# skywaLKer518/A-Recsys

Measured on AMD Instinct MI355X. Metric: training interactions/sec + sampled-negatives/sec, dim-128, 1/2/4/8 MI355X, higher is better.
Workload: dtype f32; 1 GPU; C3 (BASELINE configs[2]): id feature + multi-hot category attribute, HET layout (two tables, ~20 tokens/item over 100 k rows); synthetic 1000000-item/1000000-user HMF, dim 128, WMRB 'mw' loss, 1024 shared negatives/step (pool redrawn on device every 50 step...; batch=16384, n_sampled=1024, dim=128, n_items=1000000, hipgraph=True, ids_fed_from=HBM (device-resident ring of batches)

## Files before the change

### a-recsys_amd/csrc/scorer.hip

```cpp
#include "common.h"
#include "posmask.h"

namespace arx {

namespace {

typedef __bf16 bf16x8 __attribute__((ext_vector_type(8)));
typedef float f32x16 __attribute__((ext_vector_type(16)));

#ifndef SC_TRACE_CHUNKS
#define SC_TRACE_CHUNKS 0
#endif
#ifdef SC_TRACE
__device__ unsigned long long g_sc_trace[4096];
#define SC_T(ev_)                                                                                        \
  if (blockIdx.x == (gridDim.x > 5 ? 5 : 0) && threadIdx.x == 0 && tcount < 4096)                        \
    g_sc_trace[tcount++] = ((unsigned long long)(ev_) << 56) | (__builtin_readcyclecounter() & 0xFFFFFFFFFFFFFFull);
#define SC_TDECL int tcount = 0;
#define SC_TREAL(ev_)                  \
  if (blockIdx.x == (gridDim.x > 5 ? 5 : 0) && threadIdx.x == 0 && tcount < 4096)                        \
    g_sc_trace[tcount++] = ((unsigned long long)(ev_) << 56) | (__builtin_amdgcn_s_memrealtime() & 0xFFFFFFFFFFFFFFull);
#else
#define SC_TREAL(ev_)
#define SC_T(ev_)
#define SC_TDECL
#endif
constexpr int kScHits = 8;
constexpr int kScSlots = 4;
constexpr int kScAhead = 3;
constexpr int kScStageBytes = 3 * 32 * 256;

typedef __bf16 sc_bf2 __attribute__((ext_vector_type(2)));
typedef float sc_f2 __attribute__((ext_vector_type(2)));
__device__ __forceinline__ void split3x2(float x, float y, uint32_t& p1, uint32_t& p2, uint32_t& p3) {
  p1 = __builtin_bit_cast(uint32_t, __builtin_convertvector((sc_f2){x, y}, sc_bf2));
  const float rx = x - __uint_as_float(p1 << 16), ry = y - __uint_as_float(p1 & 0xFFFF0000u);
  p2 = __builtin_bit_cast(uint32_t, __builtin_convertvector((sc_f2){rx, ry}, sc_bf2));
  const float sx = rx - __uint_as_float(p2 << 16), sy = ry - __uint_as_float(p2 & 0xFFFF0000u);
  p3 = __builtin_bit_cast(uint32_t, __builtin_convertvector((sc_f2){sx, sy}, sc_bf2));
}

#ifdef SC_ABL_NOBAR
// ... 91 lines not shown
}

__device__ __forceinline__ float sc_wsum(float v) {
#pragma unroll
  for (int o = 32; o > 0; o >>= 1) v += __shfl_xor(v, o, 64);
  return v;
}

struct ScTScore {
  const float* U; int64_t ldu;
  const float* T; int64_t ldt;
  const float* tb; int64_t tb_stride;
  float* tscore; float* tscore2;
};

template <bool MASKS>
__global__ __launch_bounds__(256) void k_sc_prep(const float* __restrict__ P, int64_t ldp, int64_t S, int d,
                                                 const float* __restrict__ pbias, uint16_t* __restrict__ Pp,
                                                 uint16_t* __restrict__ PT, int64_t ldpt, float* __restrict__ pool_bad,
                                                 PosMask pm,
                                                 int64_t mask_rows, int64_t B, int32_t* __restrict__ hits,
                                                 int32_t* __restrict__ nhit, const float* __restrict__ seq_w,
                                                 int64_t seq_rows, float* __restrict__ row_w_out, ScTScore ts,
                                                 uint32_t* __restrict__ maskR, int64_t ldr) {
  __shared__ float tile[32 * 129];
  __shared__ float sbad[4];
  const int tid = threadIdx.x;
  const int64_t pblocks = S / 32;
  const int64_t hblocks = (B + 7) / 8;
  if ((int64_t)blockIdx.x >= pblocks + hblocks) {
    float* part = tile;
    const int cx = tid & 31, ty = tid >> 5;
    const int64_t b = ((int64_t)blockIdx.x - pblocks - hblocks) * 32 + cx;
    const int64_t L = B / seq_rows;
    float sum = 0.f;
    if (b < seq_rows)
      for (int64_t t = ty; t < L; t += 8) sum += seq_w[t * seq_rows + b];
// ... 28 lines not shown
    __syncthreads();
    if (tid == 0) pool_bad[blockIdx.x] = (sbad[0] + sbad[1]) + (sbad[2] + sbad[3]);
    sc_emit_planes_t(tile, ld, 32, d, PT, (int64_t)d * ldpt, ldpt, r0, tid, 256);
    return;
  }
  const int lane = tid & 63, hl = lane & 31;
  const int64_t r = (((int64_t)blockIdx.x - pblocks) * 256 + tid) >> 5;
  const bool valid = r < B;
  float4 u4 = make_float4(0.f, 0.f, 0.f, 0.f), t4 = u4;
  if (valid && 4 * hl < d) {
    u4 = *reinterpret_cast<const float4*>(ts.U + r * ts.ldu + 4 * hl);
    t4 = *reinterpret_cast<const float4*>(ts.T + r * ts.ldt + 4 * hl);
  }
  const float tbv = (valid && ts.tb) ? ts.tb[r * ts.tb_stride] : 0.f;
  const bool walker = valid && r < mask_rows;
  const int64_t reps = walker ? (B - r + mask_rows - 1) / mask_rows : 0;
  const int usr = walker ? pm.user_ids[r % mask_rows] : 0;
  const int beg = walker ? pm.pos_ptr[usr] : 0, end = walker ? pm.pos_ptr[usr + 1] : 0;
  int n = 0;
  uint32_t mw0 = 0u, mw1 = 0u;
  for (int p0 = beg;; p0 += 32) {
    const bool active = p0 < end && (MASKS || n >= 0);
    if (!__any(active)) break;
    const int p = p0 + hl;
    int j = -1;
    if (active && p < end) {
      j = pos_slot(pm, pm.pos_items[p]);
      if (j < 0 || j >= S) j = -1;
    }
    const unsigned long long hm64 = __ballot(j >= 0);
    uint32_t hm = (lane >> 5) ? (uint32_t)(hm64 >> 32) : (uint32_t)hm64;
    if (MASKS) {
      while (__any(hm != 0u)) {
        const bool some = hm != 0u;
        const int srcl = some ? __builtin_ctz(hm) : 0;
        hm &= hm - 1u;
        const int jj = __shfl(j, (lane & 32) + srcl, 64);
        if (some && hl == ((jj >> 5) & 31)) {
          if (jj < 1024) mw0 |= 1u << (jj & 31);
          else mw1 |= 1u << (jj & 31);
        }
      }
    } else {
      const int k = __popc(hm);
      if (active && n >= 0) {
        if (n + k > kScHits) n = -1;
        else {
          if (j >= 0) {
            const int at = n + __popc(hm & ((1u << hl) - 1u));
            for (int64_t t = 0; t < reps; ++t) hits[(r + t * mask_rows) * kScHits + at] = j;
          }
          n += k;
        }
      }
    }
  }
  if (MASKS && walker) {
    const int nwords = (int)(S >> 5);
    if (hl < nwords) maskR[(int64_t)hl * ldr + r] = mw0;
    if (hl + 32 < nwords) maskR[(int64_t)(hl + 32) * ldr + r] = mw1;
  }
  float dot = u4.x * t4.x + u4.y * t4.y + u4.z * t4.z + u4.w * t4.w;
#pragma unroll
  for (int o = 16; o > 0; o >>= 1) dot += __shfl_xor(dot, o, 64);
  if (!MASKS && hl == 0)
    for (int64_t t = 0; t < reps; ++t) nhit[r + t * mask_rows] = n;
  if (hl == 0 && valid) {
    const float t = dot + tbv;
    ts.tscore[r] = t;
    if (ts.tscore2) ts.tscore2[r] = t;
  }
}

template <int KD>
__global__ __launch_bounds__(512) void k_sc_hinge(int64_t B, int64_t S, int CW, const float* __restrict__ U, int64_t ldu,
                                                  const float* __restrict__ tscore,
                                                  const uint16_t* __restrict__ Pp, const float* __restrict__ bias,
                                                  uint32_t* __restrict__ bits, int64_t ldbits, float* __restrict__ rs_part,
                                                  float* __restrict__ cnt_part) {
  constexpr int NCH = KD / 16;
  constexpr int ROWB = KD * 2;
  constexpr int TPS = 256 / ROWB;
  constexpr int TILEB = 3 * 32 * ROWB;
  extern __shared__ __attribute__((aligned(1024))) char lds[];
  float* sbias = reinterpret_cast<float*>(lds + kScSlots * kScStageBytes);
  uint32_t* swords = reinterpret_cast<uint32_t*>(sbias + CW);
  const int tid = threadIdx.x;
  const int lane = tid & 63;
  const int wv = tid >> 6;
  const int nsplit = (int)(S / CW);
  int64_t rb;
  int ch;
// ... 18 lines not shown
    sc_loader_loop<ROWB>(ld, lds, nstage);
    return;
  }

  const int lr = lane & 31, kg = lane >> 5;
  const int64_t row = rb * 128 + wv * 32 + lr;
  const bool ok = row < B;
  SC_TDECL
  SC_TREAL(120)
  SC_T(99)
  bf16x8 a1[NCH], a2[NCH], a3[NCH];
  float4 ru[NCH][2];
  float tm1;
  {
    float bv[2];
#pragma unroll
    for (int k = 0; k < 2; ++k) bv[k] = (bias && tid + 256 * k < CW) ? bias[col0 + tid + 256 * k] : 0.f;
    tm1 = (ok ? tscore[row] : 0.f) - 1.f;
    const float* up = U + (ok ? row : 0) * ldu + 8 * kg;
#pragma unroll
    for (int c = 0; c < NCH; ++c) {
      ru[c][0] = *reinterpret_cast<const float4*>(up + 16 * c);
      ru[c][1] = *reinterpret_cast<const float4*>(up + 16 * c + 4);
      if (c & 1) __builtin_amdgcn_sched_barrier(0);
    }
#pragma unroll
    for (int k = 0; k < 2; ++k)
      if (tid + 256 * k < CW) sbias[tid + 256 * k] = bv[k];
  }
#define SC_SPLIT(c_)                                                                                     \
  {                                                                                                      \
    uint32_t p1[4], p2[4], p3[4];                                                                        \
    split3x2(ru[c_][0].x, ru[c_][0].y, p1[0], p2[0], p3[0]);                                             \
    split3x2(ru[c_][0].z, ru[c_][0].w, p1[1], p2[1], p3[1]);                                             \
    split3x2(ru[c_][1].x, ru[c_][1].y, p1[2], p2[2], p3[2]);                                             \
    split3x2(ru[c_][1].z, ru[c_][1].w, p1[3], p2[3], p3[3]);                                             \
    a1[c_] = __builtin_bit_cast(bf16x8, make_uint4(p1[0], p1[1], p1[2], p1[3]));                         \
    a2[c_] = __builtin_bit_cast(bf16x8, make_uint4(p2[0], p2[1], p2[2], p2[3]));                         \
    a3[c_] = __builtin_bit_cast(bf16x8, make_uint4(p3[0], p3[1], p3[2], p3[3]));                         \
  }
  SC_SPLIT(0)
  float rs = 0.f;
  int cnt = 0;
  constexpr bool FA1 = ROWB == 256;
  uint32_t fa[FA1 ? 1 : NCH];
#pragma unroll
  for (int c = 0; c < (FA1 ? 1 : NCH); ++c) fa[c] = (uint32_t)(lr * ROWB + 16 * ((2 * c + kg) ^ sc_swz<ROWB>(lr)));
#define SC_FA(c_) (FA1 ? (fa[0] ^ (uint32_t)((c_) << 5)) : fa[FA1 ? 0 : (c_)])

  f32x16 hiA, loA, hiB, loB;
  constexpr int VPC = 16 / NCH;
  constexpr int VPM = KD == 128 ? 2 : 4;
  uint32_t* wptr = swords + wv * 32 + lr;
  uint4 fr[4][3];
  float4 bvn[4];
  uint32_t h = 0u;
  float zero_v;
  asm volatile("v_mov_b32 %0, 0" : "=v"(zero_v));
#ifndef SC_PF
#define SC_PF 1
#endif
  static_assert(SC_PF == 1 || !FA1, "the single address register steps to the next image one chunk ahead");
#define SC_LD3(set_, c_)                                                                                 \
  {                                                                                                      \
    const uint32_t fa_ = SC_FA(c_);                                                                      \
    fr[set_][0] = *reinterpret_cast<const uint4*>(lds + fa_);                                            \
    fr[set_][1] = *reinterpret_cast<const uint4*>(lds + fa_ + 32 * ROWB);                                \
    fr[set_][2] = *reinterpret_cast<const uint4*>(lds + fa_ + 64 * ROWB);                                \
  }
#define SC_MFMA6(hi_, lo_, c_)                                                                           \
  lo_ = SC_MFMA(b3, a1[c_], lo_);                                                                        \
  hi_ = SC_MFMA(b1, a1[c_], hi_);                                                                        \
  lo_ = SC_MFMA(b1, a3[c_], lo_);                                                                        \
  lo_ = SC_MFMA(b2, a2[c_], lo_);                                                                        \
  lo_ = SC_MFMA(b2, a1[c_], lo_);                                                                        \
  lo_ = SC_MFMA(b1, a2[c_], lo_);
#define SC_WORD(hw_, j_)                                                                                 \
  {                                                                                                      \
    const uint32_t hh = (hw_) & 0xFFFFu;                                                                 \
    cnt += __popc(hh);                                                                                   \
    const uint32_t w = ((hh & 0xFu) | ((hh & 0xF0u) << 4) | ((hh & 0xF00u) << 8) | ((hh & 0xF000u) << 12)) << (4 * kg); \
    const auto sw = __builtin_amdgcn_permlane32_swap(w, w, false, false);                                \
    wptr[(j_) * 128] = sw[0] | sw[1];                                                                    \
  }
#ifdef SC_ABL_NOEPI
#define SC_EPI_ON(x_) false
#else
#define SC_EPI_ON(x_) (x_)
#endif
#ifndef SC_EPI_C0
#define SC_EPI_C0 0
#endif
#ifndef SC_EPI_V
#define SC_EPI_V VPC
#endif
#ifdef SC_ABL_EPI_NOREAD
#define SC_EPI_READ(x_) (bvn[i >> 2].x + tm1)
#else
// ... 16 lines not shown
    __builtin_amdgcn_sched_group_barrier(0x008, 2, 0);                                                   \
  }
#else
#define SC_CHUNK_SCHED(c_)                                                                               \
  _Pragma("unroll") for (int m = 0; m < 6; ++m) {                                                        \
    __builtin_amdgcn_sched_group_barrier(0x008, 1, 0);                                                   \
    if ((c_) == 0) __builtin_amdgcn_sched_group_barrier(0x002, VPM + 3, 0);                              \
    else __builtin_amdgcn_sched_group_barrier(0x002, VPM, 0);                                            \
  }
#endif
#define SC_CHUNK_SCHED_PRO                                                                               \
  _Pragma("unroll") for (int m = 0; m < 6; ++m) {                                                        \
    __builtin_amdgcn_sched_group_barrier(0x008, 1, 0);                                                   \
    __builtin_amdgcn_sched_group_barrier(0x002, 8, 0);                                                   \
  }
#define SC_TILE(hi_, lo_, hy_, ly_, EPI_, PRO_, jw_, jb0_, jb_, dl_, BAR_)                               \
  {                                                                                                      \
    const uint32_t dl = (uint32_t)(dl_);                                                                 \
    _Pragma("unroll") for (int c = 0; c < NCH; ++c) {                                                    \
      if ((BAR_) && c == NCH / 2) sc_barrier();                                                          \
      const bf16x8 b1 = __builtin_bit_cast(bf16x8, fr[c % 4][0]), b2 = __builtin_bit_cast(bf16x8, fr[c % 4][1]), \
                   b3 = __builtin_bit_cast(bf16x8, fr[c % 4][2]);                                        \
      if (FA1 && c == NCH - 1) fa[0] += dl;         \
      SC_LD3((c + SC_PF) % 4, (c + SC_PF) % NCH)    \
       \
       \
                         \
      _Pragma("unroll") for (int g = 0; g < 4; ++g) {                                                    \
        const int lastc = SC_EPI_C0 + (15 - 4 * g) / SC_EPI_V;           \
        if (lastc + 1 < NCH ? c == lastc + 1 : c == 0)                                                   \
          bvn[g] = *reinterpret_cast<const float4*>(sbias + (lastc + 1 < NCH ? (jb_) : (jb0_)) * 32 + 4 * kg + 8 * g); \
      }                                                                                                  \
      __builtin_amdgcn_sched_barrier(0);                                                                 \
      SC_MFMA6(hi_, lo_, c)                                                                              \
      if (!FA1) fa[FA1 ? 0 : c] += dl;                                                                   \
      if (c == 0 && (jw_) >= 0) {                                                                        \
        const uint32_t hw = h;                                                                           \
        SC_WORD(hw, jw_)                                                                                 \
      }                                                                                                  \
      if (SC_EPI_ON(EPI_) && c >= SC_EPI_C0 && c < SC_EPI_C0 + 16 / SC_EPI_V) {                          \
        _Pragma("unroll") for (int q = 0; q < SC_EPI_V; ++q) {                                           \
          const int i = 15 - ((c - SC_EPI_C0) * SC_EPI_V + q);                                           \
          const float nv = SC_EPI_READ(-hy_[i] - ly_[i]);                                                \
          h = __builtin_amdgcn_alignbit(h, __float_as_uint(nv), 31);                                     \
          rs += fmaxf(-nv, 0.f);                                                                         \
          const float4 bq = bvn[i >> 2];                                                                 \
          SC_EPI_WRITE(hy_[i] = ((i & 3) == 0 ? bq.x : (i & 3) == 1 ? bq.y : (i & 3) == 2 ? bq.z : bq.w) - tm1;) \
          SC_EPI_WRITE({ float z_; asm volatile("v_mov_b32 %0, 0" : "=v"(z_)); ly_[i] = z_; })          \
        }                                                                                                \
      }                                                                                                  \
      if ((PRO_) && c + 1 < NCH) { SC_SPLIT(c + 1) }                                                     \
      if (PRO_) { SC_CHUNK_SCHED_PRO } else { SC_CHUNK_SCHED(c) }                                        \
      __builtin_amdgcn_sched_barrier(0);                                                                 \
      if (SC_TRACE_CHUNKS || c == NCH - 1) { SC_T(1 + c) }                                               \
    }                                                                                                    \
  }
#define SC_INIT(hi_, lo_, j_)                                                                            \
  {                                                                                                      \
    const float* bt = sbias + (j_) * 32 + 4 * kg;                                                        \
    _Pragma("unroll") for (int g = 0; g < 4; ++g) {                                                      \
      const float4 bv = *reinterpret_cast<const float4*>(bt + 8 * g);                                    \
      hi_[4 * g] = bv.x - tm1; hi_[4 * g + 1] = bv.y - tm1; hi_[4 * g + 2] = bv.z - tm1; hi_[4 * g + 3] = bv.w - tm1; \
    }                                                                                                    \
    _Pragma("unroll") for (int e = 0; e < 16; ++e) lo_[e] = zero_v;                                      \
  }
  auto img = [&](int j) -> int { return ((j / TPS) % kScSlots) * kScStageBytes + (j % TPS) * TILEB; };
  auto step = [&](int j) -> int { return img(j + 1) - img(j); };
  SC_T(100)
  sc_barrier();
  SC_T(101)
  SC_INIT(hiA, loA, 0)
  SC_INIT(hiB, loB, 1)
#pragma unroll
  for (int c = 0; c < SC_PF; ++c) SC_LD3(c, c)
  auto tcl = [&](int j) -> int { return j < ntile ? j : ntile - 1; };
  SC_TILE(hiA, loA, hiB, loB, false, true, -1, tcl(1), tcl(2), step(0), TPS == 1)
  SC_TILE(hiB, loB, hiA, loA, true, false, -1, tcl(2), tcl(3), step(1), true)
  for (int j = 2; j + 1 < ntile; j += 2) {
    SC_TILE(hiA, loA, hiB, loB, true, false, j - 2, tcl(j + 1), tcl(j + 2), step(j), TPS == 1)
    SC_TILE(hiB, loB, hiA, loA, true, false, j - 1, tcl(j + 2), tcl(j + 3), step(j + 1), true)
  }
  SC_WORD(h, ntile - 2)
#pragma unroll
  for (int i = 15; i >= 0; --i) {
    const float nv = -hiB[i] - loB[i];
    h = __builtin_amdgcn_alignbit(h, __float_as_uint(nv), 31);
    rs += fmaxf(-nv, 0.f);
  }
  SC_WORD(h, ntile - 1)
  SC_T(110)
  asm volatile("s_waitcnt lgkmcnt(0)" ::: "memory");
  if (ok) {
    for (int j = kg; j < ntile; j += 2) bits[(col0 / 32 + j) * ldbits + row] = swords[j * 128 + wv * 32 + lr];
  }
  SC_T(111)
  SC_TREAL(121)
#undef SC_LD3
#undef SC_SPLIT
#undef SC_MFMA6
#undef SC_TILE
#undef SC_WORD
#undef SC_INIT
  rs += __shfl_xor(rs, 32, 64);
  cnt += __shfl_xor(cnt, 32, 64);
  if (kg == 0 && ok) {
    rs_part[(int64_t)ch * B + row] = rs;
    cnt_part[(int64_t)ch * B + row] = (float)cnt;
  }
}

struct ScRows {
  const float* rs_part;
  const float* cnt_part;
  int nsplit;
  uint32_t* bits;
  int64_t ldbits;
  uint32_t* bitsT; int64_t ldbt;
  const float* tscore;
  const float* U; int64_t ldu;
  const float* T; int64_t ldt;
  const float* P; int64_t ldp;
  const float* pb;
  int d;
  float gscale;
  const float* row_w;
  float* batch_loss;
  float* g_out;
  float* dtscore; int64_t dts_stride;
  float* dU; int64_t lddu;
  float* dT; int64_t lddt;
  uint16_t* UgT; int64_t ldug;
  float* dbp;
  const int32_t* hits;
  const int32_t* nhit;
  const float* pool_bad;
};

template <int LPR>
__global__ __launch_bounds__(512) void k_sc_rows_g(ScRows a, PosMask pm, int64_t mask_rows, int64_t B, int64_t S) {
  constexpr int G = 64 / LPR;
  constexpr int WPL = 64 / LPR;
  constexpr int ROUNDS = 4 / G;
  static_assert(G == 2 || G == 4, "d = 128 or d = 64");
  __shared__ float tile[32 * 129];
  __shared__ uint32_t sbits[32 * 64];
  __shared__ float sg[32];
  const int tid = threadIdx.x;
  const int lane = tid & 63;
  const int wv = tid >> 6;
  const int j = lane % LPR, grp = lane / LPR, gbase = grp * LPR;
  const int64_t r0 = (int64_t)blockIdx.x * 32;
  const int nwords = (int)(S >> 5);
  const int ld = a.d + 1;
  const float pbad = sc_wsum(lane < nwords ? a.pool_bad[lane] : 0.f);
  auto gsum = [](float v) {
#pragma unroll
    for (int o = LPR / 2; o > 0; o >>= 1) v += __shfl_xor(v, o, 64);
    return v;
  };
#pragma unroll
  for (int it = 0; it < ROUNDS; ++it) {
    const int rl = wv * 4 + it * G + grp;
    const int64_t r = r0 + rl;
    const bool live = r < B;
    float4 uq = make_float4(0.f, 0.f, 0.f, 0.f), tq = uq;
    float sq = 0.f, cq = 0.f, t = 0.f;
    int nh = 0;
    uint32_t w[WPL], w0[WPL];
#pragma unroll
    for (int k = 0; k < WPL; ++k) w[k] = 0u;
    if (live) {
      for (int p = 0; p < a.nsplit; ++p) {
        sq += a.rs_part[(int64_t)p * B + r];
        cq += a.cnt_part[(int64_t)p * B + r];
      }
      t = a.tscore[r];
      uq = *reinterpret_cast<const float4*>(a.U + r * a.ldu + j * 4);
      tq = *reinterpret_cast<const float4*>(a.T + r * a.ldt + j * 4);
      nh = a.nhit[r];
#pragma unroll
      for (int k = 0; k < WPL; ++k)
        if (k * LPR + j < nwords) w[k] = a.bits[(int64_t)(k * LPR + j) * a.ldbits + r];
    }
#pragma unroll
    for (int k = 0; k < WPL; ++k) w0[k] = w[k];
    if (__any(live && nh != 0)) {
      auto take_out = [&](int jj, bool act) {
        const int wi = jj >> 5, own = wi % LPR, slot = wi / LPR;
        uint32_t mine = w[0];
#pragma unroll
        for (int k = 1; k < WPL; ++k) mine = slot == k ? w[k] : mine;
        const uint32_t word = __shfl(mine, gbase + own, 64);
        const bool on = act && ((word >> (jj & 31)) & 1u);
        float4 pr = make_float4(0.f, 0.f, 0.f, 0.f);
        if (on) pr = *reinterpret_cast<const float4*>(a.P + (int64_t)jj * a.ldp + j * 4);
        const float x = gsum(uq.x * pr.x + uq.y * pr.y + uq.z * pr.z + uq.w * pr.w) + ((on && a.pb) ? a.pb[jj] : 0.f);
        const float v = x - t + 1.f;
        if (on) {
          sq -= v > 0.f ? v : 0.f;
          cq -= 1.f;
          if (j == own) {
#pragma unroll
            for (int k = 0; k < WPL; ++k)
              if (slot == k) w[k] &= ~(1u << (jj & 31));
          }
        }
      };
      const bool listed = live && nh > 0;
      const int myhit = (listed && j < nh) ? a.hits[r * kScHits + j] : 0;
      for (int k = 0; k < kScHits; ++k) {
        const bool act = listed && k < nh;
        if (!__any(act)) break;
        take_out(__shfl(myhit, gbase + k, 64), act);
      }
      const bool walk = live && nh < 0;
      if (__any(walk)) {
        const int usr = walk ? pm.user_ids[r % mask_rows] : 0;
        const int beg = walk ? pm.pos_ptr[usr] : 0, end = walk ? pm.pos_ptr[usr + 1] : 0;
        for (int p0 = beg;; p0 += LPR) {
          const bool more = walk && p0 < end;
          if (!__any(more)) break;
          const int p = p0 + j;
          int js = -1;
          if (more && p < end) {
            js = pos_slot(pm, pm.pos_items[p]);
            if (js < 0 || js >= S) js = -1;
          }
          const unsigned long long bal = __ballot(js >= 0);
          uint32_t hm = (uint32_t)((bal >> gbase) & ((LPR == 32) ? 0xffffffffull : 0xffffull));
          while (__any(hm != 0u)) {
            const bool act = hm != 0u;
            const int src = act ? __builtin_ctz(hm) : 0;
            hm &= hm - 1u;
            take_out(__shfl(js, gbase + src, 64), act);
          }
        }
      }
      if (live && nh != 0) {
#pragma unroll
        for (int k = 0; k < WPL; ++k)
          if (k * LPR + j < nwords && w[k] != w0[k]) a.bits[(int64_t)(k * LPR + j) * a.ldbits + r] = w[k];
      }
    }
    sq = fmaxf(sq, 0.f) + (pbad + gsum(((uq.x + uq.y) + (uq.z + uq.w) + (tq.x + tq.y) + (tq.z + tq.w)) * 0.f) + t * 0.f);
    const float g = live ? a.gscale * (a.row_w ? a.row_w[r] : 1.f) / (1.f + sq) : 0.f;
    const float dt = -g * cq;
    if (j == 0) {
      sg[rl] = g;
      if (live) {
        if (a.batch_loss) a.batch_loss[r] = logf(1.f + sq);
        if (a.dtscore) a.dtscore[r * a.dts_stride] = dt;
      }
      a.g_out[r] = g;
    }
#pragma unroll
    for (int k = 0; k < WPL; ++k)
      if (k * LPR + j < nwords) sbits[rl * 64 + k * LPR + j] = w[k];
// ... 690 lines not shown
    float* tp = tile + rl * (D + 1) + c4;
    const float cu = live ? coef : 0.f;
    tp[0] = cu * u.x; tp[1] = cu * u.y; tp[2] = cu * u.z; tp[3] = cu * u.w;
  }
  __syncthreads();
  sc_emit_planes_t(tile, D + 1, 32, D, a.UgT, (int64_t)D * a.ldug, a.ldug, r0, tid, 256);
}


}

struct ScLayout {
  int64_t Bp, ldbits, ldbt, nblk;
  int64_t ldpt, ldug;
  int nsplit, CW;
  size_t bits, bitsT, g, t, rs, cnt, hits, nhit, Pp, PT, UgT, dbp, pbad, total;
};

static bool sc_layout(int64_t B, int64_t S, int d, ScLayout* L) {
  if (!(d == 64 || d == 128) || S % 128 != 0 || S < 128 || S > 2048 || B < 1) return false;
  L->Bp = (B + 127) / 128 * 128;
  L->ldbits = (B + 255) / 256 * 256;
  L->ldbt = (S + 255) / 256 * 256;
  L->nblk = L->Bp / 32;
  L->ldpt = S + 128;
  L->ldug = L->Bp + 128;
  L->CW = S >= 1024 ? 512 : (S >= 256 ? (int)(S / 2) : (int)S);
  L->nsplit = (int)(S / L->CW);
  size_t o = 0;
  auto take = [&](size_t bytes) { const size_t at = o; o += al256(bytes); return at; };
  L->bits = take((size_t)(S / 32) * L->ldbits * 4);
  L->bitsT = take((size_t)L->nblk * L->ldbt * 4);
  L->g = take((size_t)L->Bp * 4);
  L->t = take((size_t)B * 4);
  L->rs = take((size_t)L->nsplit * B * 4);
  L->cnt = take((size_t)L->nsplit * B * 4);
  L->hits = take((size_t)B * kScHits * 4);
  L->nhit = take((size_t)B * 4);
  L->Pp = take((size_t)3 * S * d * 2);
  L->PT = take((size_t)3 * d * L->ldpt * 2);
  L->UgT = take((size_t)3 * d * L->ldug * 2);
  L->dbp = take((size_t)L->nblk * S * 4);
  L->pbad = take(64 * 4);
  L->total = o;
  return true;
}

static int sc_raise_lds() {
  const int cap = 160 * 1024;
  ARX_CHECK_HIP(hipFuncSetAttribute(reinterpret_cast<const void*>(k_sc_hinge<128>), hipFuncAttributeMaxDynamicSharedMemorySize, cap));
  ARX_CHECK_HIP(hipFuncSetAttribute(reinterpret_cast<const void*>(k_sc_hinge<64>), hipFuncAttributeMaxDynamicSharedMemorySize, cap));
  ARX_CHECK_HIP(hipFuncSetAttribute(reinterpret_cast<const void*>(k_sc_bits<false>), hipFuncAttributeMaxDynamicSharedMemorySize, cap));
  ARX_CHECK_HIP(hipFuncSetAttribute(reinterpret_cast<const void*>(k_sc_bits<true>), hipFuncAttributeMaxDynamicSharedMemorySize, cap));
  return ARX_OK;
}

}

// ... 47 lines not shown
  if (!ok) {
    set_error("arx_mw_scorer_fwd: shape not supported (d in {64, 128}, S %% 128 == 0, 128 <= S <= 2048, 16-byte rows)");
    return ARX_EUNSUPPORTED;
  }
  if (state_bytes < L.total) {
    set_error("arx_mw_scorer_fwd: state too small (%zu < %zu)", state_bytes, L.total);
    return ARX_EWORKSPACE;
  }
  if (int rc = sc_raise_lds()) return rc;
  hipStream_t s = as_stream(stream);
  char* st = reinterpret_cast<char*>(state);
  uint32_t* bits = reinterpret_cast<uint32_t*>(st + L.bits);
  float* t = reinterpret_cast<float*>(st + L.t);
  float* rs_part = reinterpret_cast<float*>(st + L.rs);
  float* cnt_part = reinterpret_cast<float*>(st + L.cnt);
  int32_t* hits = reinterpret_cast<int32_t*>(st + L.hits);
  int32_t* nhit = reinterpret_cast<int32_t*>(st + L.nhit);
  uint16_t* Pp = reinterpret_cast<uint16_t*>(st + L.Pp);
  uint16_t* PT = reinterpret_cast<uint16_t*>(st + L.PT);
  const PosMask pm = make_pos_mask(user_ids, pos_ptr, pos_items, item2slot);
  const int64_t mrows = mask_rows > 0 ? mask_rows : B;
  if (phases & 1) {
    const int64_t grid = S / 32 + ceil_div(B, 8) + (seq_w ? ceil_div(seq_rows, 32) : 0);
    const ScTScore ts{U, ldu, T, ldt, tbias, tb_stride > 0 ? tb_stride : 1, t, tscore_out};
    k_sc_prep<false><<<(int)grid, 256, 0, s>>>(P, ldp, S, d, pbias, Pp, PT, L.ldpt, reinterpret_cast<float*>(st + L.pbad),
                                               pm, mrows, B, hits, nhit, seq_w, seq_rows, row_w, ts, nullptr, 0);
    ARX_CHECK_LAUNCH();
  }
  if (phases & 2) {
    const int64_t grid = ceil_div(B, 128) * L.nsplit;
    const size_t lds = (size_t)kScSlots * kScStageBytes + (size_t)L.CW * 4 + (size_t)(L.CW / 32) * 128 * 4;
    if (d == 128)
      k_sc_hinge<128><<<(int)grid, 512, lds, s>>>(B, S, L.CW, U, ldu, t, Pp, pbias, bits, L.ldbits, rs_part, cnt_part);
    else
      k_sc_hinge<64><<<(int)grid, 512, lds, s>>>(B, S, L.CW, U, ldu, t, Pp, pbias, bits, L.ldbits, rs_part, cnt_part);
    ARX_CHECK_LAUNCH();
  }
  if (phases & 4) {
    ScRows a{rs_part, cnt_part, L.nsplit, bits, L.ldbits, reinterpret_cast<uint32_t*>(st + L.bitsT), L.ldbt, t, U, ldu, T, ldt,
             P, ldp, pbias, d, gscale, row_w, batch_loss, reinterpret_cast<float*>(st + L.g), dtscore,
             dtscore_stride > 0 ? dtscore_stride : 1, dU, lddu, dT, lddt, reinterpret_cast<uint16_t*>(st + L.UgT), L.ldug,
             reinterpret_cast<float*>(st + L.dbp), hits, nhit, reinterpret_cast<const float*>(st + L.pbad)};
    if (d == 64) k_sc_rows_g<16><<<(int)L.nblk, 512, 0, s>>>(a, pm, mrows, B, S);
    else k_sc_rows_g<32><<<(int)L.nblk, 512, 0, s>>>(a, pm, mrows, B, S);
    ARX_CHECK_LAUNCH();
  }
  return ARX_OK;
}

int arx_mw_scorer_bwd_du(int64_t B, int64_t S, int d, const void* state, float beta, float* dU, int64_t lddu,
                         void* stream) {
  ScLayout L;
  ARX_CHECK_ARG(state && dU && sc_layout(B, S, d, &L), "arx_mw_scorer_bwd_du: bad argument / shape");
  ARX_CHECK_ARG(lddu % 4 == 0 && lddu >= d && (reinterpret_cast<uintptr_t>(dU) & 15) == 0,
                "arx_mw_scorer_bwd_du: dU rows must be 16-byte aligned");
  if (int rc = sc_raise_lds()) return rc;
  const char* st = reinterpret_cast<const char*>(state);
  const int64_t grid = ceil_div(B, 256) * (d / 32);
  k_sc_bits<false><<<(int)grid, 512, (size_t)kScSlots * (kScStageBytes + 4096), as_stream(stream)>>>(
// ... 62 lines not shown
      part, (int)nsl, S, d, beta, dI, lddi, dbp, L.nblk, db, dbblocks, batch_loss, row_w, B, gscale, loss_out,
      stepblocks, bps, Lsteps, db_steps);
  ARX_CHECK_LAUNCH();
  return ARX_OK;
}

}

namespace arx {
namespace {

struct McLayout {
  int64_t Bp, ldpt, ldug, ldr;
  int nsplit;
  int64_t CW;
  size_t maskR, mask_bytes, t, tneg, coef, rs, O, hits, nhit, Pp, PT, Up, UgT, pbad, zeros, total;
};

bool mc_layout(int64_t B, int64_t S, int d, McLayout* L) {
  if (!(d == 64 || d == 128) || S % 128 != 0 || S < 128 || S > 2048 || B < 1) return false;
  L->Bp = (B + 127) / 128 * 128;
  L->ldpt = S + 128;
  L->ldug = L->Bp + 128;
  L->ldr = L->Bp;
  int ns = 1;
  while (ns < 4 && (L->Bp / 128) * ns < 3 * (int64_t)cu_count() && S / (2 * ns) >= 128 && (S / (2 * ns)) % 32 == 0) ns *= 2;
  L->nsplit = ns;
  L->CW = S / ns;
  size_t o = 0;
  auto take = [&](size_t bytes) { const size_t at = o; o += al256(bytes); return at; };
  L->maskR = take((size_t)(S / 32) * L->ldr * 4);
  L->mask_bytes = o;
  L->t = take((size_t)B * 4);
  L->tneg = take((size_t)L->Bp * 4);
  L->coef = take((size_t)L->Bp * 4);
  L->rs = take((size_t)ns * B * 4);
  L->O = take((size_t)ns * L->Bp * d * 4);
  L->hits = take((size_t)B * kScHits * 4);
  L->nhit = take((size_t)B * 4);
  L->Pp = take((size_t)3 * S * d * 2);
  L->PT = take((size_t)3 * d * L->ldpt * 2);
  L->Up = take((size_t)3 * L->Bp * d * 2);
  L->UgT = take((size_t)3 * d * L->ldug * 2);
  L->pbad = take(64 * 4);
  L->zeros = take(256);
  L->total = o;
  return true;
}

int mc_raise_lds() {
  ARX_CHECK_HIP(hipFuncSetAttribute(reinterpret_cast<const void*>(k_mc_flow<false, 64>), hipFuncAttributeMaxDynamicSharedMemorySize, 80 * 1024));
  ARX_CHECK_HIP(hipFuncSetAttribute(reinterpret_cast<const void*>(k_mc_flow<true, 64>), hipFuncAttributeMaxDynamicSharedMemorySize, 80 * 1024));
  ARX_CHECK_HIP(hipFuncSetAttribute(reinterpret_cast<const void*>(k_mc_flow<false, 128>), hipFuncAttributeMaxDynamicSharedMemorySize, 152 * 1024));
  ARX_CHECK_HIP(hipFuncSetAttribute(reinterpret_cast<const void*>(k_mc_flow<true, 128>), hipFuncAttributeMaxDynamicSharedMemorySize, 152 * 1024));
// ... 51 lines not shown
                "arx_mce_scorer_fwd: mask_rows must be B or a multiple of 128 that divides B");
  if (int rc = mc_raise_lds()) return rc;
  hipStream_t s = as_stream(stream);
  char* st = reinterpret_cast<char*>(state);
  float* t = reinterpret_cast<float*>(st + L.t);
  uint16_t* Pp = reinterpret_cast<uint16_t*>(st + L.Pp);
  uint16_t* PT = reinterpret_cast<uint16_t*>(st + L.PT);
  uint32_t* maskR = reinterpret_cast<uint32_t*>(st + L.maskR);
  float* rs_part = reinterpret_cast<float*>(st + L.rs);
  float* O_part = reinterpret_cast<float*>(st + L.O);
  const PosMask pm = make_pos_mask(user_ids, pos_ptr, pos_items, item2slot);
  const int64_t mrows = mask_rows > 0 ? mask_rows : B;
  if (phases & 1) {
    const int64_t grid = S / 32 + ceil_div(B, 8) + (seq_w ? ceil_div(seq_rows, 32) : 0);
    const ScTScore ts{U, ldu, T, ldt, tbias, tb_stride > 0 ? tb_stride : 1, t, tscore_out};
    k_sc_prep<true><<<(int)grid, 256, 0, s>>>(P, ldp, S, d, pbias, Pp, PT, L.ldpt, reinterpret_cast<float*>(st + L.pbad),
                                              pm, mrows, B, reinterpret_cast<int32_t*>(st + L.hits),
                                              reinterpret_cast<int32_t*>(st + L.nhit), seq_w, seq_rows, row_w, ts,
                                              maskR, L.ldr);
    ARX_CHECK_LAUNCH();
  }
  if (phases & 2) {
    McFlow a{};
    a.nstat = B; a.span = L.CW; a.nstream = S;
    a.statF = U; a.ldstat = ldu;
    a.XK = Pp; a.xk_plane = S * d;
    a.XT = PT; a.ldx = L.ldpt;
    a.cstat = t; a.sgn_stat = -1.f;
    a.cstream = pbias; a.cw = nullptr;
    a.mask = maskR; a.ldmask = L.ldr;
    a.mask_mod = mrows;
    a.zeros = reinterpret_cast<const float*>(st + L.zeros);
    a.O = O_part; a.o_rows = L.Bp;
    a.rsum = rs_part; a.rs_rows = B;
// ... 83 lines not shown
```

Before: 72.06 million interactions/s.

## Fold positive-item masking into hinge kernel via bitmask instead of rows-pass correction

The scorer prep kernel now always builds a per-row positive-slot bitmask (maskR) rather than a small hit list with a walk fallback. The hinge kernel loads these mask words and seeds the low accumulator with a large negative value for masked columns, so positives are excluded inside the MFMA epilogue. This removes the correction pass in the rows kernel that re-dotted each positive against P and patched the bit words. In exchange it adds mask loads, doubles the LDS word buffer, and relies on the large-negative trick to keep those columns out of the hinge.

```diff
diff --git a/a-recsys_amd/csrc/scorer.hip b/a-recsys_amd/csrc/scorer.hip
--- a/a-recsys_amd/csrc/scorer.hip
+++ b/a-recsys_amd/csrc/scorer.hip
@@ -25,7 +25,6 @@
 #define SC_T(ev_)
 #define SC_TDECL
 #endif
-constexpr int kScHits = 8;
 constexpr int kScSlots = 4;
 constexpr int kScAhead = 3;
 constexpr int kScStageBytes = 3 * 32 * 256;
@@ -147,13 +146,11 @@
   float* tscore; float* tscore2;
 };
 
-template <bool MASKS>
 __global__ __launch_bounds__(256) void k_sc_prep(const float* __restrict__ P, int64_t ldp, int64_t S, int d,
                                                  const float* __restrict__ pbias, uint16_t* __restrict__ Pp,
                                                  uint16_t* __restrict__ PT, int64_t ldpt, float* __restrict__ pool_bad,
                                                  PosMask pm,
-                                                 int64_t mask_rows, int64_t B, int32_t* __restrict__ hits,
-                                                 int32_t* __restrict__ nhit, const float* __restrict__ seq_w,
+                                                 int64_t mask_rows, int64_t B, const float* __restrict__ seq_w,
                                                  int64_t seq_rows, float* __restrict__ row_w_out, ScTScore ts,
                                                  uint32_t* __restrict__ maskR, int64_t ldr) {
   __shared__ float tile[32 * 129];
@@ -212,13 +209,11 @@
   }
   const float tbv = (valid && ts.tb) ? ts.tb[r * ts.tb_stride] : 0.f;
   const bool walker = valid && r < mask_rows;
-  const int64_t reps = walker ? (B - r + mask_rows - 1) / mask_rows : 0;
   const int usr = walker ? pm.user_ids[r % mask_rows] : 0;
   const int beg = walker ? pm.pos_ptr[usr] : 0, end = walker ? pm.pos_ptr[usr + 1] : 0;
-  int n = 0;
   uint32_t mw0 = 0u, mw1 = 0u;
   for (int p0 = beg;; p0 += 32) {
-    const bool active = p0 < end && (MASKS || n >= 0);
+    const bool active = p0 < end;
     if (!__any(active)) break;
     const int p = p0 + hl;
     int j = -1;
@@ -228,32 +223,18 @@
     }
     const unsigned long long hm64 = __ballot(j >= 0);
     uint32_t hm = (lane >> 5) ? (uint32_t)(hm64 >> 32) : (uint32_t)hm64;
-    if (MASKS) {
-      while (__any(hm != 0u)) {
-        const bool some = hm != 0u;
-        const int srcl = some ? __builtin_ctz(hm) : 0;
-        hm &= hm - 1u;
-        const int jj = __shfl(j, (lane & 32) + srcl, 64);
-        if (some && hl == ((jj >> 5) & 31)) {
-          if (jj < 1024) mw0 |= 1u << (jj & 31);
-          else mw1 |= 1u << (jj & 31);
-        }
+    while (__any(hm != 0u)) {
+      const bool some = hm != 0u;
+      const int srcl = some ? __builtin_ctz(hm) : 0;
+      hm &= hm - 1u;
+      const int jj = __shfl(j, (lane & 32) + srcl, 64);
+      if (some && hl == ((jj >> 5) & 31)) {
+        if (jj < 1024) mw0 |= 1u << (jj & 31);
+        else mw1 |= 1u << (jj & 31);
       }
-    } else {
-      const int k = __popc(hm);
-      if (active && n >= 0) {
-        if (n + k > kScHits) n = -1;
-        else {
-          if (j >= 0) {
-            const int at = n + __popc(hm & ((1u << hl) - 1u));
-            for (int64_t t = 0; t < reps; ++t) hits[(r + t * mask_rows) * kScHits + at] = j;
-          }
-          n += k;
-        }
-      }
-    }
-  }
-  if (MASKS && walker) {
+    }
+  }
+  if (walker) {
     const int nwords = (int)(S >> 5);
     if (hl < nwords) maskR[(int64_t)hl * ldr + r] = mw0;
     if (hl + 32 < nwords) maskR[(int64_t)(hl + 32) * ldr + r] = mw1;
@@ -261,8 +242,6 @@
   float dot = u4.x * t4.x + u4.y * t4.y + u4.z * t4.z + u4.w * t4.w;
 #pragma unroll
   for (int o = 16; o > 0; o >>= 1) dot += __shfl_xor(dot, o, 64);
-  if (!MASKS && hl == 0)
-    for (int64_t t = 0; t < reps; ++t) nhit[r + t * mask_rows] = n;
   if (hl == 0 && valid) {
     const float t = dot + tbv;
     ts.tscore[r] = t;
@@ -274,6 +253,7 @@
 __global__ __launch_bounds__(512) void k_sc_hinge(int64_t B, int64_t S, int CW, const float* __restrict__ U, int64_t ldu,
                                                   const float* __restrict__ tscore,
                                                   const uint16_t* __restrict__ Pp, const float* __restrict__ bias,
+                                                  const uint32_t* __restrict__ maskR, int64_t ldr, int64_t mask_rows,
                                                   uint32_t* __restrict__ bits, int64_t ldbits, float* __restrict__ rs_part,
                                                   float* __restrict__ cnt_part) {
   constexpr int NCH = KD / 16;
@@ -322,9 +302,15 @@
   float tm1;
   {
     float bv[2];
+    uint32_t mv[8];
 #pragma unroll
     for (int k = 0; k < 2; ++k) bv[k] = (bias && tid + 256 * k < CW) ? bias[col0 + tid + 256 * k] : 0.f;
     tm1 = (ok ? tscore[row] : 0.f) - 1.f;
+    int64_t mrow = row;
+    if (row >= mask_rows) mrow = (B >> 31) == 0 ? (int64_t)((uint32_t)row % (uint32_t)mask_rows) : row % mask_rows;
+    const uint32_t* mp = maskR + (col0 / 32 + kg) * ldr + mrow;
+#pragma unroll
+    for (int k = 0; k < 8; ++k) mv[k] = (ok && kg + 2 * k < ntile) ? mp[(int64_t)2 * k * ldr] : 0u;
     const float* up = U + (ok ? row : 0) * ldu + 8 * kg;
 #pragma unroll
     for (int c = 0; c < NCH; ++c) {
@@ -335,6 +321,12 @@
 #pragma unroll
     for (int k = 0; k < 2; ++k)
       if (tid + 256 * k < CW) sbias[tid + 256 * k] = bv[k];
+#pragma unroll
+    for (int k = 0; k < 8; ++k)
+      if (kg + 2 * k < ntile) {
+        swords[(kg + 2 * k) * 256 + wv * 64 + lr] = mv[k];
+        swords[(kg + 2 * k) * 256 + wv * 64 + 32 + lr] = mv[k] >> 4;
+      }
   }
 #define SC_SPLIT(c_)                                                                                     \
   {                                                                                                      \
@@ -359,12 +351,18 @@
   f32x16 hiA, loA, hiB, loB;
   constexpr int VPC = 16 / NCH;
   constexpr int VPM = KD == 128 ? 2 : 4;
-  uint32_t* wptr = swords + wv * 32 + lr;
+  uint32_t* wptr = swords + wv * 64 + lane;
   uint4 fr[4][3];
   float4 bvn[4];
   uint32_t h = 0u;
-  float zero_v;
-  asm volatile("v_mov_b32 %0, 0" : "=v"(zero_v));
+  uint32_t mkA = 0u, mkB = 0u;
+#define SC_LO0(m_, i_)                                                                                   \
+  ({                                                                                                     \
+    float z_;                                                                                            \
+    asm volatile("v_bfe_i32 %0, %1, %2, 1\n\tv_and_b32 %0, 0xf149f2ca, %0"                                \
+                 : "=v"(z_) : "v"(m_), "n"(8 * ((i_) >> 2) + ((i_) & 3)));                               \
+    z_;                                                                                                  \
+  })
 #ifndef SC_PF
 #define SC_PF 1
 #endif
@@ -389,7 +387,7 @@
     cnt += __popc(hh);                                                                                   \
     const uint32_t w = ((hh & 0xFu) | ((hh & 0xF0u) << 4) | ((hh & 0xF00u) << 8) | ((hh & 0xF000u) << 12)) << (4 * kg); \
     const auto sw = __builtin_amdgcn_permlane32_swap(w, w, false, false);                                \
-    wptr[(j_) * 128] = sw[0] | sw[1];                                                                    \
+    wptr[(j_) * 256] = sw[0] | sw[1];                                                                    \
   }
 #ifdef SC_ABL_NOEPI
 #define SC_EPI_ON(x_) false
@@ -436,14 +434,18 @@
     __builtin_amdgcn_sched_group_barrier(0x008, 1, 0);                                                   \
     __builtin_amdgcn_sched_group_barrier(0x002, 8, 0);                                                   \
   }
-#define SC_TILE(hi_, lo_, hy_, ly_, EPI_, PRO_, jw_, jb0_, jb_, dl_, BAR_)                               \
+#define SC_TILE(hi_, lo_, hy_, ly_, mu_, ml_, EPI_, PRO_, jw_, jb0_, jb_, dl_, BAR_)                     \
+   \
   {                                                                                                      \
     const uint32_t dl = (uint32_t)(dl_);                                                                 \
     _Pragma("unroll") for (int c = 0; c < NCH; ++c) {                                                    \
       if ((BAR_) && c == NCH / 2) sc_barrier();                                                          \
       const bf16x8 b1 = __builtin_bit_cast(bf16x8, fr[c % 4][0]), b2 = __builtin_bit_cast(bf16x8, fr[c % 4][1]), \
                    b3 = __builtin_bit_cast(bf16x8, fr[c % 4][2]);                                        \
-      if (FA1 && c == NCH - 1) fa[0] += dl;         \
+      if (FA1 && c == NCH - 1) {                    \
+        fa[0] += dl;                                \
+        asm volatile("" : "+v"(fa[0]));             \
+      }                                                                                                  \
       SC_LD3((c + SC_PF) % 4, (c + SC_PF) % NCH)    \
        \
        \
@@ -453,6 +455,7 @@
         if (lastc + 1 < NCH ? c == lastc + 1 : c == 0)                                                   \
           bvn[g] = *reinterpret_cast<const float4*>(sbias + (lastc + 1 < NCH ? (jb_) : (jb0_)) * 32 + 4 * kg + 8 * g); \
       }                                                                                                  \
+      if (c == NCH - 1) ml_ = wptr[(jb_) * 256];                                                         \
       __builtin_amdgcn_sched_barrier(0);                                                                 \
       SC_MFMA6(hi_, lo_, c)                                                                              \
       if (!FA1) fa[FA1 ? 0 : c] += dl;                                                                   \
@@ -468,7 +471,7 @@
           rs += fmaxf(-nv, 0.f);                                                                         \
           const float4 bq = bvn[i >> 2];                                                                 \
           SC_EPI_WRITE(hy_[i] = ((i & 3) == 0 ? bq.x : (i & 3) == 1 ? bq.y : (i & 3) == 2 ? bq.z : bq.w) - tm1;) \
-          SC_EPI_WRITE({ float z_; asm volatile("v_mov_b32 %0, 0" : "=v"(z_)); ly_[i] = z_; })          \
+          SC_EPI_WRITE(ly_[i] = SC_LO0(mu_, i);)                                                         \
         }                                                                                                \
       }                                                                                                  \
       if ((PRO_) && c + 1 < NCH) { SC_SPLIT(c + 1) }                                                     \
@@ -484,7 +487,8 @@
       const float4 bv = *reinterpret_cast<const float4*>(bt + 8 * g);                                    \
       hi_[4 * g] = bv.x - tm1; hi_[4 * g + 1] = bv.y - tm1; hi_[4 * g + 2] = bv.z - tm1; hi_[4 * g + 3] = bv.w - tm1; \
     }                                                                                                    \
-    _Pragma("unroll") for (int e = 0; e < 16; ++e) lo_[e] = zero_v;                                      \
+    const uint32_t m0_ = wptr[(j_) * 256];                                                               \
+    _Pragma("unroll") for (int e = 0; e < 16; ++e) lo_[e] = SC_LO0(m0_, e);                              \
   }
   auto img = [&](int j) -> int { return ((j / TPS) % kScSlots) * kScStageBytes + (j % TPS) * TILEB; };
   auto step = [&](int j) -> int { return img(j + 1) - img(j); };
@@ -493,14 +497,15 @@
   SC_T(101)
   SC_INIT(hiA, loA, 0)
   SC_INIT(hiB, loB, 1)
+  __builtin_amdgcn_sched_barrier(0);
 #pragma unroll
   for (int c = 0; c < SC_PF; ++c) SC_LD3(c, c)
   auto tcl = [&](int j) -> int { return j < ntile ? j : ntile - 1; };
-  SC_TILE(hiA, loA, hiB, loB, false, true, -1, tcl(1), tcl(2), step(0), TPS == 1)
-  SC_TILE(hiB, loB, hiA, loA, true, false, -1, tcl(2), tcl(3), step(1), true)
+  SC_TILE(hiA, loA, hiB, loB, mkB, mkA, false, true, -1, tcl(1), tcl(2), step(0), TPS == 1)
+  SC_TILE(hiB, loB, hiA, loA, mkA, mkB, true, false, -1, tcl(2), tcl(3), step(1), true)
   for (int j = 2; j + 1 < ntile; j += 2) {
-    SC_TILE(hiA, loA, hiB, loB, true, false, j - 2, tcl(j + 1), tcl(j + 2), step(j), TPS == 1)
-    SC_TILE(hiB, loB, hiA, loA, true, false, j - 1, tcl(j + 2), tcl(j + 3), step(j + 1), true)
+    SC_TILE(hiA, loA, hiB, loB, mkB, mkA, true, false, j - 2, tcl(j + 1), tcl(j + 2), step(j), TPS == 1)
+    SC_TILE(hiB, loB, hiA, loA, mkA, mkB, true, false, j - 1, tcl(j + 2), tcl(j + 3), step(j + 1), true)
   }
   SC_WORD(h, ntile - 2)
 #pragma unroll
@@ -513,7 +518,7 @@
   SC_T(110)
   asm volatile("s_waitcnt lgkmcnt(0)" ::: "memory");
   if (ok) {
-    for (int j = kg; j < ntile; j += 2) bits[(col0 / 32 + j) * ldbits + row] = swords[j * 128 + wv * 32 + lr];
+    for (int j = kg; j < ntile; j += 2) bits[(col0 / 32 + j) * ldbits + row] = wptr[j * 256];
   }
   SC_T(111)
   SC_TREAL(121)
@@ -523,6 +528,7 @@
 #undef SC_TILE
 #undef SC_WORD
 #undef SC_INIT
+#undef SC_LO0
   rs += __shfl_xor(rs, 32, 64);
   cnt += __shfl_xor(cnt, 32, 64);
   if (kg == 0 && ok) {
@@ -535,14 +541,12 @@
   const float* rs_part;
   const float* cnt_part;
   int nsplit;
-  uint32_t* bits;
+  const uint32_t* bits;
   int64_t ldbits;
   uint32_t* bitsT; int64_t ldbt;
   const float* tscore;
   const float* U; int64_t ldu;
   const float* T; int64_t ldt;
-  const float* P; int64_t ldp;
-  const float* pb;
   int d;
   float gscale;
   const float* row_w;
@@ -553,13 +557,11 @@
   float* dT; int64_t lddt;
   uint16_t* UgT; int64_t ldug;
   float* dbp;
-  const int32_t* hits;
-  const int32_t* nhit;
   const float* pool_bad;
 };
 
 template <int LPR>
-__global__ __launch_bounds__(512) void k_sc_rows_g(ScRows a, PosMask pm, int64_t mask_rows, int64_t B, int64_t S) {
+__global__ __launch_bounds__(512) void k_sc_rows_g(ScRows a, int64_t B, int64_t S) {
   constexpr int G = 64 / LPR;
   constexpr int WPL = 64 / LPR;
   constexpr int ROUNDS = 4 / G;
@@ -587,8 +589,7 @@
     const bool live = r < B;
     float4 uq = make_float4(0.f, 0.f, 0.f, 0.f), tq = uq;
     float sq = 0.f, cq = 0.f, t = 0.f;
-    int nh = 0;
-    uint32_t w[WPL], w0[WPL];
+    uint32_t w[WPL];
 #pragma unroll
     for (int k = 0; k < WPL; ++k) w[k] = 0u;
     if (live) {
@@ -599,70 +600,9 @@
       t = a.tscore[r];
       uq = *reinterpret_cast<const float4*>(a.U + r * a.ldu + j * 4);
       tq = *reinterpret_cast<const float4*>(a.T + r * a.ldt + j * 4);
-      nh = a.nhit[r];
 #pragma unroll
       for (int k = 0; k < WPL; ++k)
         if (k * LPR + j < nwords) w[k] = a.bits[(int64_t)(k * LPR + j) * a.ldbits + r];
-    }
-#pragma unroll
-    for (int k = 0; k < WPL; ++k) w0[k] = w[k];
-    if (__any(live && nh != 0)) {
-      auto take_out = [&](int jj, bool act) {
-        const int wi = jj >> 5, own = wi % LPR, slot = wi / LPR;
-        uint32_t mine = w[0];
-#pragma unroll
-        for (int k = 1; k < WPL; ++k) mine = slot == k ? w[k] : mine;
-        const uint32_t word = __shfl(mine, gbase + own, 64);
-        const bool on = act && ((word >> (jj & 31)) & 1u);
-        float4 pr = make_float4(0.f, 0.f, 0.f, 0.f);
-        if (on) pr = *reinterpret_cast<const float4*>(a.P + (int64_t)jj * a.ldp + j * 4);
-        const float x = gsum(uq.x * pr.x + uq.y * pr.y + uq.z * pr.z + uq.w * pr.w) + ((on && a.pb) ? a.pb[jj] : 0.f);
-        const float v = x - t + 1.f;
-        if (on) {
-          sq -= v > 0.f ? v : 0.f;
-          cq -= 1.f;
-          if (j == own) {
-#pragma unroll
-            for (int k = 0; k < WPL; ++k)
-              if (slot == k) w[k] &= ~(1u << (jj & 31));
-          }
-        }
-      };
-      const bool listed = live && nh > 0;
-      const int myhit = (listed && j < nh) ? a.hits[r * kScHits + j] : 0;
-      for (int k = 0; k < kScHits; ++k) {
-        const bool act = listed && k < nh;
-        if (!__any(act)) break;
-        take_out(__shfl(myhit, gbase + k, 64), act);
-      }
-      const bool walk = live && nh < 0;
-      if (__any(walk)) {
-        const int usr = walk ? pm.user_ids[r % mask_rows] : 0;
-        const int beg = walk ? pm.pos_ptr[usr] : 0, end = walk ? pm.pos_ptr[usr + 1] : 0;
-        for (int p0 = beg;; p0 += LPR) {
-          const bool more = walk && p0 < end;
-          if (!__any(more)) break;
-          const int p = p0 + j;
-          int js = -1;
-          if (more && p < end) {
-            js = pos_slot(pm, pm.pos_items[p]);
-            if (js < 0 || js >= S) js = -1;
-          }
-          const unsigned long long bal = __ballot(js >= 0);
-          uint32_t hm = (uint32_t)((bal >> gbase) & ((LPR == 32) ? 0xffffffffull : 0xffffull));
-          while (__any(hm != 0u)) {
-            const bool act = hm != 0u;
-            const int src = act ? __builtin_ctz(hm) : 0;
-            hm &= hm - 1u;
-            take_out(__shfl(js, gbase + src, 64), act);
-          }
-        }
-      }
-      if (live && nh != 0) {
-#pragma unroll
-        for (int k = 0; k < WPL; ++k)
-          if (k * LPR + j < nwords && w[k] != w0[k]) a.bits[(int64_t)(k * LPR + j) * a.ldbits + r] = w[k];
-      }
     }
     sq = fmaxf(sq, 0.f) + (pbad + gsum(((uq.x + uq.y) + (uq.z + uq.w) + (tq.x + tq.y) + (tq.z + tq.w)) * 0.f) + t * 0.f);
     const float g = live ? a.gscale * (a.row_w ? a.row_w[r] : 1.f) / (1.f + sq) : 0.f;
@@ -1383,7 +1323,8 @@
   int64_t Bp, ldbits, ldbt, nblk;
   int64_t ldpt, ldug;
   int nsplit, CW;
-  size_t bits, bitsT, g, t, rs, cnt, hits, nhit, Pp, PT, UgT, dbp, pbad, total;
+  int64_t ldr;
+  size_t bits, bitsT, g, t, rs, cnt, Pp, PT, UgT, dbp, pbad, maskR, total;
 };
 
 static bool sc_layout(int64_t B, int64_t S, int d, ScLayout* L) {
@@ -1404,13 +1345,13 @@
   L->t = take((size_t)B * 4);
   L->rs = take((size_t)L->nsplit * B * 4);
   L->cnt = take((size_t)L->nsplit * B * 4);
-  L->hits = take((size_t)B * kScHits * 4);
-  L->nhit = take((size_t)B * 4);
   L->Pp = take((size_t)3 * S * d * 2);
   L->PT = take((size_t)3 * d * L->ldpt * 2);
   L->UgT = take((size_t)3 * d * L->ldug * 2);
   L->dbp = take((size_t)L->nblk * S * 4);
   L->pbad = take(64 * 4);
+  L->ldr = L->Bp;
+  L->maskR = take((size_t)(S / 32) * L->ldr * 4);
   L->total = o;
   return true;
 }
@@ -1488,8 +1429,7 @@
   float* t = reinterpret_cast<float*>(st + L.t);
   float* rs_part = reinterpret_cast<float*>(st + L.rs);
   float* cnt_part = reinterpret_cast<float*>(st + L.cnt);
-  int32_t* hits = reinterpret_cast<int32_t*>(st + L.hits);
-  int32_t* nhit = reinterpret_cast<int32_t*>(st + L.nhit);
+  uint32_t* maskR = reinterpret_cast<uint32_t*>(st + L.maskR);
   uint16_t* Pp = reinterpret_cast<uint16_t*>(st + L.Pp);
   uint16_t* PT = reinterpret_cast<uint16_t*>(st + L.PT);
   const PosMask pm = make_pos_mask(user_ids, pos_ptr, pos_items, item2slot);
@@ -1497,26 +1437,28 @@
   if (phases & 1) {
     const int64_t grid = S / 32 + ceil_div(B, 8) + (seq_w ? ceil_div(seq_rows, 32) : 0);
     const ScTScore ts{U, ldu, T, ldt, tbias, tb_stride > 0 ? tb_stride : 1, t, tscore_out};
-    k_sc_prep<false><<<(int)grid, 256, 0, s>>>(P, ldp, S, d, pbias, Pp, PT, L.ldpt, reinterpret_cast<float*>(st + L.pbad),
-                                               pm, mrows, B, hits, nhit, seq_w, seq_rows, row_w, ts, nullptr, 0);
+    k_sc_prep<<<(int)grid, 256, 0, s>>>(P, ldp, S, d, pbias, Pp, PT, L.ldpt, reinterpret_cast<float*>(st + L.pbad), pm,
+                                        mrows, B, seq_w, seq_rows, row_w, ts, maskR, L.ldr);
     ARX_CHECK_LAUNCH();
   }
   if (phases & 2) {
     const int64_t grid = ceil_div(B, 128) * L.nsplit;
-    const size_t lds = (size_t)kScSlots * kScStageBytes + (size_t)L.CW * 4 + (size_t)(L.CW / 32) * 128 * 4;
+    const size_t lds = (size_t)kScSlots * kScStageBytes + (size_t)L.CW * 4 + (size_t)(L.CW / 32) * 256 * 4;
     if (d == 128)
-      k_sc_hinge<128><<<(int)grid, 512, lds, s>>>(B, S, L.CW, U, ldu, t, Pp, pbias, bits, L.ldbits, rs_part, cnt_part);
+      k_sc_hinge<128><<<(int)grid, 512, lds, s>>>(B, S, L.CW, U, ldu, t, Pp, pbias, maskR, L.ldr, mrows, bits, L.ldbits,
+                                                  rs_part, cnt_part);
     else
-      k_sc_hinge<64><<<(int)grid, 512, lds, s>>>(B, S, L.CW, U, ldu, t, Pp, pbias, bits, L.ldbits, rs_part, cnt_part);
+      k_sc_hinge<64><<<(int)grid, 512, lds, s>>>(B, S, L.CW, U, ldu, t, Pp, pbias, maskR, L.ldr, mrows, bits, L.ldbits,
+                                                 rs_part, cnt_part);
     ARX_CHECK_LAUNCH();
   }
   if (phases & 4) {
     ScRows a{rs_part, cnt_part, L.nsplit, bits, L.ldbits, reinterpret_cast<uint32_t*>(st + L.bitsT), L.ldbt, t, U, ldu, T, ldt,
-             P, ldp, pbias, d, gscale, row_w, batch_loss, reinterpret_cast<float*>(st + L.g), dtscore,
+             d, gscale, row_w, batch_loss, reinterpret_cast<float*>(st + L.g), dtscore,
              dtscore_stride > 0 ? dtscore_stride : 1, dU, lddu, dT, lddt, reinterpret_cast<uint16_t*>(st + L.UgT), L.ldug,
-             reinterpret_cast<float*>(st + L.dbp), hits, nhit, reinterpret_cast<const float*>(st + L.pbad)};
-    if (d == 64) k_sc_rows_g<16><<<(int)L.nblk, 512, 0, s>>>(a, pm, mrows, B, S);
-    else k_sc_rows_g<32><<<(int)L.nblk, 512, 0, s>>>(a, pm, mrows, B, S);
+             reinterpret_cast<float*>(st + L.dbp), reinterpret_cast<const float*>(st + L.pbad)};
+    if (d == 64) k_sc_rows_g<16><<<(int)L.nblk, 512, 0, s>>>(a, B, S);
+    else k_sc_rows_g<32><<<(int)L.nblk, 512, 0, s>>>(a, B, S);
     ARX_CHECK_LAUNCH();
   }
   return ARX_OK;
@@ -1609,7 +1551,7 @@
   int64_t Bp, ldpt, ldug, ldr;
   int nsplit;
   int64_t CW;
-  size_t maskR, mask_bytes, t, tneg, coef, rs, O, hits, nhit, Pp, PT, Up, UgT, pbad, zeros, total;
+  size_t maskR, mask_bytes, t, tneg, coef, rs, O, Pp, PT, Up, UgT, pbad, zeros, total;
 };
 
 bool mc_layout(int64_t B, int64_t S, int d, McLayout* L) {
@@ -1631,8 +1573,6 @@
   L->coef = take((size_t)L->Bp * 4);
   L->rs = take((size_t)ns * B * 4);
   L->O = take((size_t)ns * L->Bp * d * 4);
-  L->hits = take((size_t)B * kScHits * 4);
-  L->nhit = take((size_t)B * 4);
   L->Pp = take((size_t)3 * S * d * 2);
   L->PT = take((size_t)3 * d * L->ldpt * 2);
   L->Up = take((size_t)3 * L->Bp * d * 2);
@@ -1714,10 +1654,8 @@
   if (phases & 1) {
     const int64_t grid = S / 32 + ceil_div(B, 8) + (seq_w ? ceil_div(seq_rows, 32) : 0);
     const ScTScore ts{U, ldu, T, ldt, tbias, tb_stride > 0 ? tb_stride : 1, t, tscore_out};
-    k_sc_prep<true><<<(int)grid, 256, 0, s>>>(P, ldp, S, d, pbias, Pp, PT, L.ldpt, reinterpret_cast<float*>(st + L.pbad),
-                                              pm, mrows, B, reinterpret_cast<int32_t*>(st + L.hits),
-                                              reinterpret_cast<int32_t*>(st + L.nhit), seq_w, seq_rows, row_w, ts,
-                                              maskR, L.ldr);
+    k_sc_prep<<<(int)grid, 256, 0, s>>>(P, ldp, S, d, pbias, Pp, PT, L.ldpt, reinterpret_cast<float*>(st + L.pbad), pm,
+                                        mrows, B, seq_w, seq_rows, row_w, ts, maskR, L.ldr);
     ARX_CHECK_LAUNCH();
   }
   if (phases & 2) {
```

Measured after the change: 72.23 million interactions/s, median of 3. Within noise of the previous version (+0.2%).
